# hrnr/map-merge

Hardware: NVIDIA B200
Metric: pairwise_registrations_per_sec (higher is better)
Workload: dtype f32

## Files before the change

map-merge_b200/csrc/icp.cu:

```cuda
#include <algorithm>
#include <cmath>
#include <cstring>
#include <type_traits>

#include "mm3d_internal.cuh"

namespace mm3d {

namespace {

constexpr int IB = 128;
constexpr int NSUM = 17;

struct IcpState {
  float final_t[16];
  float step[16];
  double prev_mse;
  int iterations;
  int active;
  int converged;
  int pad;
};

struct IcpJob {
  GridView tgt;
  ReachView reach;
  const float4* src;
  int ns;
  float4* work;
  long long* sums;
  IcpState* st;
  int* ticket;
  int* next_tile;
  int n_tiles;
  float t0[16];
  long long* sums_log;
  int* nn_slot;
};

struct IcpLoop {
  int n_active;
  int pad[3];
};

struct ReachJob {
  GridView g;
  ReachView r;
  unsigned char* a;
  unsigned char* b;
};

__global__ void __launch_bounds__(256) reach_mark_kernel(const ReachJob* __restrict__ jobs)
{
  const ReachJob& j = jobs[blockIdx.y];
  for (int i = blockIdx.x * blockDim.x + threadIdx.x; i < j.g.n; i += gridDim.x * blockDim.x) {
    const float4 p = j.g.pts[i];
    const int x = floor_to_int(p.x * j.g.inv_leaf) - j.g.min_b[0] - j.r.org[0];
    const int y = floor_to_int(p.y * j.g.inv_leaf) - j.g.min_b[1] - j.r.org[1];
    const int z = floor_to_int(p.z * j.g.inv_leaf) - j.g.min_b[2] - j.r.org[2];
    if (x >= 0 && y >= 0 && z >= 0 && x < j.r.dim[0] && y < j.r.dim[1] && z < j.r.dim[2])
      j.a[((size_t)z * j.r.dim[1] + y) * j.r.dim[0] + x] = 0;
  }
}

__global__ void __launch_bounds__(256) reach_pass_kernel(const ReachJob* __restrict__ jobs, int axis, int margin, int from_a)
{
  const ReachJob& j = jobs[blockIdx.y];
  const size_t ncell = (size_t)j.r.dim[0] * j.r.dim[1] * j.r.dim[2];
  const unsigned char* in = from_a ? j.a : j.b;
  unsigned char* out = from_a ? j.b : j.a;
  for (size_t c = (size_t)blockIdx.x * blockDim.x + threadIdx.x; c < ncell; c += (size_t)gridDim.x * blockDim.x) {
    const int x = (int)(c % j.r.dim[0]);
    const int y = (int)((c / j.r.dim[0]) % j.r.dim[1]);
    const int z = (int)(c / ((size_t)j.r.dim[0] * j.r.dim[1]));
    const int pos = axis == 0 ? x : (axis == 1 ? y : z);
    const int len = j.r.dim[axis];
    const long long stride = axis == 0 ? 1 : (axis == 1 ? (long long)j.r.dim[0] : (long long)j.r.dim[0] * j.r.dim[1]);
    const int lo = max(-margin, -pos), hi = min(margin, len - 1 - pos);
    int best = 255;
    for (int d = lo; d <= hi; ++d) {
      const int f = max(abs(d) - 1, 0);
      const int v = (int)in[(long long)c + (long long)d * stride] + f * f;
      best = min(best, v);
    }
    out[c] = (unsigned char)min(best, j.r.none);
  }
}

__device__ __forceinline__ bool reach_lookup(const GridView& g, const ReachView& r, float qx, float qy, float qz, int* lb2)
{
  const int x = floor_to_int(qx * g.inv_leaf) - g.min_b[0] - r.org[0];
  const int y = floor_to_int(qy * g.inv_leaf) - g.min_b[1] - r.org[1];
  const int z = floor_to_int(qz * g.inv_leaf) - g.min_b[2] - r.org[2];
  if (x < 0 || y < 0 || z < 0 || x >= r.dim[0] || y >= r.dim[1] || z >= r.dim[2]) return false;
  *lb2 = (int)__ldg(&r.lb2[((size_t)z * r.dim[1] + y) * r.dim[0] + x]);
  return true;
}

__device__ __forceinline__ bool reach_descend(const ReachView& r, int& x, int& y, int& z, int cur)
{
  for (int step = 0; step < 48 && cur > 0; ++step) {
    int best = cur, bx = x, by = y, bz = z;
#pragma unroll
    for (int t = 0; t < 6; ++t) {
      const int nx = x + (t == 0) - (t == 1), ny = y + (t == 2) - (t == 3), nz = z + (t == 4) - (t == 5);
      if (nx < 0 || ny < 0 || nz < 0 || nx >= r.dim[0] || ny >= r.dim[1] || nz >= r.dim[2]) continue;
      const int v = (int)__ldg(&r.lb2[((size_t)nz * r.dim[1] + ny) * r.dim[0] + nx]);
      if (v < best) {
        best = v;
        bx = nx;
        by = ny;
        bz = nz;
      }
    }
    if (best >= cur) return false;
    cur = best;
    x = bx;
    y = by;
    z = bz;
  }
  return cur == 0;
}

__device__ __forceinline__ float block27_any(const GridView& g, int vx, int vy, int vz, float qx, float qy, float qz)
{
  float best = 3.0e38f;
  const int xlo = max(vx - 1, 0), xhi = min(vx + 1, g.div_v[0] - 1);
  if (xlo > xhi) return best;
  for (int t = 0; t < 9; ++t) {
    const int cz = vz + t / 3 - 1, cy = vy + t % 3 - 1;
    if (cz < 0 || cz >= g.div_v[2] || cy < 0 || cy >= g.div_v[1]) continue;
    const int base = (cz * g.dim[1] + cy) * g.dim[0];
    const int s = __ldg(&g.cell_start[base + xlo]), e = __ldg(&g.cell_start[base + xhi + 1]);
    for (int k = s; k < e; ++k) {
      const float4 p = g.pts[k];
      best = fminf(best, em::dist2_3(qx, qy, qz, p.x, p.y, p.z));
    }
  }
  return best;
}

__device__ __forceinline__ bool nearest_block27(const GridView& g, float qx, float qy, float qz, double bound, int guess_slot, int* out_idx,
                                                float* out_d2, float4* out_pt, int* out_slot, bool* certain)
{
  const float fx = qx * g.inv_leaf, fy = qy * g.inv_leaf, fz = qz * g.inv_leaf;
  const float flx = floorf(fx), fly = floorf(fy), flz = floorf(fz);
  const int vx = (int)flx - g.min_b[0], vy = (int)fly - g.min_b[1], vz = (int)flz - g.min_b[2];
  const float ay = fy - fly, az = fz - flz;
  bool found = false;
  float best = 0.0f;
  int best_idx = 0x7fffffff, best_slot = -1;
  float4 best_pt = make_float4(0.f, 0.f, 0.f, 0.f);
  float bestv = 3.0e38f;
  const float inv2 = g.inv_leaf * g.inv_leaf;
  if (guess_slot >= 0 && guess_slot < g.n) {
    const float4 p = g.pts[guess_slot];
    const float d2 = em::dist2_3(qx, qy, qz, p.x, p.y, p.z);
    if ((double)d2 <= bound) {
      found = true;
      best = d2;
      best_idx = g.orig ? g.orig[guess_slot] : guess_slot;
      best_slot = guess_slot;
      best_pt = p;
      bestv = d2 * inv2 * 1.0001f + 1e-4f;
    }
  }
  int rs[9], re[9];
  const int xlo = max(vx - 1, 0), xhi = min(vx + 1, g.div_v[0] - 1);
  const bool x_ok = xlo <= xhi;
#pragma unroll
  for (int t = 0; t < 9; ++t) {
    const int cz = vz + t / 3 - 1, cy = vy + t % 3 - 1;
    rs[t] = 0;
    re[t] = 0;
    if (x_ok && cz >= 0 && cz < g.div_v[2] && cy >= 0 && cy < g.div_v[1]) {
      const int base = (cz * g.dim[1] + cy) * g.dim[0];
      rs[t] = __ldg(&g.cell_start[base + xlo]);
      re[t] = __ldg(&g.cell_start[base + xhi + 1]);
    }
  }
#pragma unroll
  for (int t = 0; t < 9; ++t) {
    const int dz = t / 3 - 1, dy = t % 3 - 1;
    const float zd = dz < 0 ? az : (dz > 0 ? 1.0f - az : 0.0f);
    const float yd = dy < 0 ? ay : (dy > 0 ? 1.0f - ay : 0.0f);
    if (zd * zd + yd * yd > bestv) continue;
    for (int k = rs[t]; k < re[t]; ++k) {
      const float4 p = g.pts[k];
      const float d2 = em::dist2_3(qx, qy, qz, p.x, p.y, p.z);
      if ((double)d2 > bound) continue;
      const int oi = g.orig ? g.orig[k] : k;
      if (!found || d2 < best || (d2 == best && oi < best_idx)) {
        found = true;
        best = d2;
        best_idx = oi;
        best_slot = k;
        best_pt = p;
        bestv = d2 * inv2 * 1.0001f + 1e-4f;
      }
    }
  }
  *certain = found && best * inv2 < 0.999f;
  *out_idx = best_idx;
  *out_d2 = best;
  *out_pt = best_pt;
  *out_slot = found ? best_slot : -1;
  return found;
}

struct TileNn {
  float4 q[IB];
  int todo[IB];
  int todo_large[IB];
  float res_d2[IB];
  int res_slot[IB];
  int n_todo, n_todo_large;
};

__device__ __forceinline__ bool tile_nearest(TileNn& sh, const GridView& g, const ReachView& r, bool live, float qx, float qy, float qz,
                                             double bound, int guess_slot, float* out_d2, float4* out_pt, int* out_slot)
{
  const int tid = threadIdx.x, lane = tid & 31, warp = tid >> 5;
  if (tid == 0) {
    sh.n_todo = 0;
    sh.n_todo_large = 0;
  }
  __syncthreads();
  bool hit = false, pending = false;
  float d2 = 0.f;
  int slot = -1;
  float4 pt = make_float4(0.f, 0.f, 0.f, 0.f);
  if (live) {
    float r2 = (float)bound;
    bool rejected = false, block_has_points = true;
    if (r.lb2) {
      int lb2 = 0;
      const float bound_v = (float)bound * g.inv_leaf * g.inv_leaf;
      const bool inside = reach_lookup(g, r, qx, qy, qz, &lb2);
      const float lb = inside ? (float)lb2 : (float)r.none;
      if (lb > bound_v * 1.001f + 0.01f) rejected = true;
      if (inside && lb2 < r.none) {
        const float ub = sqrtf((float)lb2) + 3.4642f;
        r2 = fminf(r2, (ub * ub * 1.001f + 0.01f) * g.leaf * g.leaf);
      }
      block_has_points = inside && lb2 == 0;
      if (!rejected && inside && lb2 > 0 && lb2 < r.none && guess_slot < 0 && g.shift[0] == 0 && g.shift[1] == 0 && g.shift[2] == 0) {
        int cx = floor_to_int(qx * g.inv_leaf) - g.min_b[0] - r.org[0];
        int cy = floor_to_int(qy * g.inv_leaf) - g.min_b[1] - r.org[1];
        int cz = floor_to_int(qz * g.inv_leaf) - g.min_b[2] - r.org[2];
        if (reach_descend(r, cx, cy, cz, lb2)) {
          const float dd = block27_any(g, cx + r.org[0], cy + r.org[1], cz + r.org[2], qx, qy, qz);
          if (dd < 3.0e38f) r2 = fminf(r2, dd);
        }
      }
    }
    if (!rejected) {
      bool certain = false;
      if ((block_has_points || guess_slot >= 0) && g.shift[0] == 0 && g.shift[1] == 0 && g.shift[2] == 0) {
        int idx;
        hit = nearest_block27(g, qx, qy, qz, bound, guess_slot, &idx, &d2, &pt, &slot, &certain);
        if (hit) r2 = fminf(r2, d2);
      }
      if (!certain) {
        pending = true;
        hit = false;
        const float r2w = r2 * 1.00001f + 1e-12f;
        sh.q[tid] = make_float4(qx, qy, qz, r2w);
        if (r2w * g.inv_leaf * g.inv_leaf <= 12.25f) sh.todo[atomicAdd(&sh.n_todo, 1)] = tid;
        else sh.todo_large[atomicAdd(&sh.n_todo_large, 1)] = tid;
      }
    }
  }
  __syncthreads();
  const int n_small = sh.n_todo, n_large = sh.n_todo_large;
  auto serve = [&](auto G_, int who, unsigned gmask, int glane) {
    constexpr int G = decltype(G_)::value;
    const float4 q = sh.q[who];
    const int rv = (int)ceilf(sqrtf(q.w) * g.inv_leaf) + 1;
    float bd = 3.0e38f;
    int bi = 0x7fffffff, bs = -1;
    group_radius_unordered<G>(g, gmask, glane, q.x, q.y, q.z, q.w, rv, [&](bool valid, int k, const float4&, float dd) {
      if (valid && (double)dd <= bound) {
        const int oi = g.orig ? g.orig[k] : k;
        if (dd < bd || (dd == bd && oi < bi)) {
          bd = dd;
          bi = oi;
          bs = k;
        }
      }
    });
#pragma unroll
    for (int o = G / 2; o > 0; o >>= 1) {
      const float od = __shfl_xor_sync(gmask, bd, o, G);
      const int oi = __shfl_xor_sync(gmask, bi, o, G);
      const int os = __shfl_xor_sync(gmask, bs, o, G);
      if (od < bd || (od == bd && oi < bi)) {
        bd = od;
        bi = oi;
        bs = os;
      }
    }
    if (glane == 0) {
      sh.res_d2[who] = bd;
      sh.res_slot[who] = bs;
    }
  };
  {
    const int grp = tid >> 3, glane = tid & 7;
    const unsigned gmask = 0xffu << (lane & 24);
    for (int t = grp; t < n_small; t += IB / 8) serve(std::integral_constant<int, 8>(), sh.todo[t], gmask, glane);
  }
  __syncwarp();
  for (int t = warp; t < n_large; t += IB / 32) serve(std::integral_constant<int, 32>(), sh.todo_large[t], 0xffffffffu, lane);
  __syncthreads();
  if (pending) {
    slot = sh.res_slot[tid];
    hit = slot >= 0;
    if (hit) {
      d2 = sh.res_d2[tid];
      pt = g.pts[slot];
    }
  }
  *out_d2 = d2;
  *out_pt = pt;
  *out_slot = hit ? slot : -1;
  return hit;
}

__global__ void __launch_bounds__(256) icp_init_kernel(const IcpJob* __restrict__ jobs)
{
  const IcpJob& j = jobs[blockIdx.y];
  for (int i = blockIdx.x * blockDim.x + threadIdx.x; i < j.ns; i += gridDim.x * blockDim.x) {
    const float4 p = j.src[i];
    float4 o;
    em::transform_point(j.t0, p.x, p.y, p.z, &o.x, &o.y, &o.z);
    o.w = p.w;
    j.work[i] = o;
    j.nn_slot[i] = -1;
  }
}

__device__ __forceinline__ void block_accumulate(long long* vals, int nvals, long long* gsums)
{
  __shared__ long long sh[IB / 32][NSUM];
  const int lane = threadIdx.x & 31, w = threadIdx.x >> 5;
  __syncthreads();
  for (int k = 0; k < nvals; ++k) {
    const long long v = warp_sum_ll(vals[k]);
    if (lane == 0) sh[w][k] = v;
  }
  __syncthreads();
  if (threadIdx.x < nvals) {
    long long s = 0;
    for (int ww = 0; ww < IB / 32; ++ww) s += sh[ww][threadIdx.x];
    if (s != 0) atomicAdd((unsigned long long*)&gsums[threadIdx.x], (unsigned long long)s);
  }
}

__device__ void mat4_mul(const float* a, const float* b, float* r)
{
  for (int i = 0; i < 4; ++i)
    for (int c = 0; c < 4; ++c) {
      float acc = a[i * 4 + 0] * b[0 * 4 + c];
      acc += a[i * 4 + 1] * b[1 * 4 + c];
      acc += a[i * 4 + 2] * b[2 * 4 + c];
      acc += a[i * 4 + 3] * b[3 * 4 + c];
      r[i * 4 + c] = acc;
    }
}

__device__ void icp_solve(const IcpJob& j, int max_iterations, double rotation_threshold, double translation_threshold, int max_log,
                          int* n_active)
{
  IcpState& st = *j.st;
  long long s[NSUM];
  for (int k = 0; k < NSUM; ++k) {
    s[k] = (long long)atomicExch((unsigned long long*)&j.sums[k], 0ull);
  }
  if (j.sums_log && st.iterations < max_log)
    for (int k = 0; k < NSUM; ++k) j.sums_log[(size_t)st.iterations * NSUM + k] = s[k];
  const long long cnt = s[0];
  if (cnt < 3) {
    st.active = 0;
    st.converged = 0;
    __threadfence();
    atomicSub(n_active, 1);
    return;
  }
  const double n = (double)cnt;
  double pm[3], qm[3];
  for (int a = 0; a < 3; ++a) {
    pm[a] = ((double)s[1 + a] / MM3D_FIX1_SCALE) / n;
    qm[a] = ((double)s[4 + a] / MM3D_FIX1_SCALE) / n;
  }
  float sigma[9], pmf[3], qmf[3];
  for (int a = 0; a < 3; ++a) {
    pmf[a] = (float)pm[a];
    qmf[a] = (float)qm[a];
    for (int b = 0; b < 3; ++b) sigma[a * 3 + b] = (float)(((double)s[7 + a * 3 + b] / MM3D_FIX2_SCALE) / n - qm[a] * pm[b]);
  }
  float T[16];
  em::umeyama_from_sigma<float>(sigma, pmf, qmf, T);
  float nf[16];
  mat4_mul(T, st.final_t, nf);
  for (int k = 0; k < 16; ++k) {
    st.final_t[k] = nf[k];
    st.step[k] = T[k];
  }
  st.iterations += 1;
  bool conv = false;
  if (st.iterations >= max_iterations) {
    conv = true;
  } else {
    const double cos_angle = 0.5 * (double)(T[0] + T[5] + T[10] - 1);
    const double translation_sqr = (double)(T[3] * T[3] + T[7] * T[7] + T[11] * T[11]);
    if (cos_angle >= rotation_threshold && translation_sqr <= translation_threshold) {
      conv = true;
    } else {
      const double mse = ((double)s[16] / MM3D_FIXD_SCALE) / n;
      if (fabs(mse - st.prev_mse) < 1e-12) conv = true;
      else st.prev_mse = mse;
    }
  }
  if (conv) {
    st.active = 0;
    st.converged = 1;
    __threadfence();
    atomicSub(n_active, 1);
  } else {
    __threadfence();
    atomicExch(j.next_tile, 0);
  }
}

__device__ __forceinline__ void icp_tile(const IcpJob& j, int tile, double max_dist_sqr, int rv, int max_iterations,
                                         double rotation_threshold, double translation_threshold, int max_log, int* n_active)
{
  __shared__ float s_step[16];
  __shared__ int s_apply;
  __shared__ TileNn nn;
  __syncthreads();
  if (threadIdx.x < 16) s_step[threadIdx.x] = __ldcg(&j.st->step[threadIdx.x]);
  if (threadIdx.x == 16) s_apply = __ldcg(&j.st->iterations) > 0 ? 1 : 0;
  __syncthreads();
  const int apply_step = s_apply;
  long long v[NSUM];
#pragma unroll
  for (int k = 0; k < NSUM; ++k) v[k] = 0;
  const int i = tile * IB + threadIdx.x;
  const bool live = i < j.ns;
  float4 p = make_float4(0.f, 0.f, 0.f, 0.f);
  int guess = -1;
  if (live) {
    p = __ldcg(&j.work[i]);
    if (apply_step) {
      float4 o;
      em::transform_point(s_step, p.x, p.y, p.z, &o.x, &o.y, &o.z);
      o.w = p.w;
      p = o;
      j.work[i] = p;
    }
    guess = __ldcg(&j.nn_slot[i]);
  }
  float d2;
  float4 q;
  int slot;
  const bool hit = tile_nearest(nn, j.tgt, j.reach, live, p.x, p.y, p.z, max_dist_sqr, guess, &d2, &q, &slot);
  if (live) {
    j.nn_slot[i] = slot;
    if (hit) {
      const double pp[3] = {(double)p.x, (double)p.y, (double)p.z};
      const double qq[3] = {(double)q.x, (double)q.y, (double)q.z};
      v[0] = 1;
#pragma unroll
      for (int a = 0; a < 3; ++a) {
        v[1 + a] = em::to_fix(pp[a], MM3D_FIX1_SCALE);
        v[4 + a] = em::to_fix(qq[a], MM3D_FIX1_SCALE);
#pragma unroll
        for (int b = 0; b < 3; ++b) v[7 + a * 3 + b] = em::to_fix(qq[a] * pp[b], MM3D_FIX2_SCALE);
      }
      v[16] = em::to_fix((double)d2, MM3D_FIXD_SCALE);
    }
  }
  block_accumulate(v, NSUM, j.sums);
  __syncthreads();
  if (threadIdx.x == 0) {
    __threadfence();
    const int ntiles = (j.ns + IB - 1) / IB;
    const int ticket = atomicAdd(j.ticket, 1);
    if (ticket == ntiles - 1) {
      *j.ticket = 0;
      __threadfence();
      icp_solve(j, max_iterations, rotation_threshold, translation_threshold, max_log, n_active);
    }
  }
}

__global__ void __launch_bounds__(IB) icp_persistent_kernel(const IcpJob* __restrict__ jobs, int n_jobs, IcpLoop* loop, double max_dist_sqr,
                                                            int rv, int max_iterations, double rotation_threshold,
                                                            double translation_threshold, int max_log)
{
  __shared__ int s_pair, s_tile;
  int cur = 0;
  for (;;) {
    if (threadIdx.x == 0) {
      int pair = -1, tile = -1, scanned = 0;
      while (__ldcg(&loop->n_active) > 0) {
        const IcpJob& j = jobs[cur];
        if (__ldcg(j.next_tile) < j.n_tiles) {
          const int t = atomicAdd(j.next_tile, 1);
          if (t < j.n_tiles) {
            __threadfence();
            pair = cur;
            tile = t;
            break;
          }
        }
        cur = cur + 1 == n_jobs ? 0 : cur + 1;
        if (++scanned >= n_jobs) {
          scanned = 0;
          __nanosleep(500);
        }
      }
      s_pair = pair;
      s_tile = tile;
    }
    __syncthreads();
    const int pair = s_pair, tile = s_tile;
    if (pair < 0) break;
    icp_tile(jobs[pair], tile, max_dist_sqr, rv, max_iterations, rotation_threshold, translation_threshold, max_log, &loop->n_active);
    __syncthreads();
  }
}

struct ScoreJob {
  GridView tgt;
  ReachView reach;
  const float4* src;
  int ns;
  float t[16];
  long long* sums;
  const int* nn_guess;
};

__global__ void __launch_bounds__(IB) score_kernel(const ScoreJob* __restrict__ jobs, double max_range, int rv)
{
  const ScoreJob& j = jobs[blockIdx.y];
  if (blockIdx.x * IB >= j.ns) return;
  __shared__ TileNn nn;
  long long v[2] = {0, 0};
  const int i = blockIdx.x * IB + threadIdx.x;
  const bool live = i < j.ns;
  float x = 0.f, y = 0.f, z = 0.f;
  if (live) {
    const float4 p = j.src[i];
    em::transform_point(j.t, p.x, p.y, p.z, &x, &y, &z);
  }
  float d2;
  float4 q;
  int slot;
  if (tile_nearest(nn, j.tgt, j.reach, live, x, y, z, max_range, (live && j.nn_guess) ? j.nn_guess[i] : -1, &d2, &q, &slot)) {
    v[0] = em::to_fix((double)d2, MM3D_FIXD_SCALE);
    v[1] = 1;
  }
  block_accumulate(v, 2, j.sums);
}

ReachView no_reach()
{
  ReachView r;
  memset(&r, 0, sizeof(r));
  return r;
}

}

void build_reach_batch(Ctx& c, const std::vector<DIndex>& idx, int margin, std::vector<DReach>& out)
{
  const int M = (int)idx.size();
  out.clear();
  out.resize(M);
  margin = std::max(2, std::min(margin, 15));
  std::vector<ReachJob> jobs;
  std::vector<DBuf<unsigned char>> ping(M);
  size_t max_cells = 0;
  int max_n = 0;
  for (int m = 0; m < M; ++m) {
    out[m].v = no_reach();
    const GridView& g = idx[m].v;
    if (g.n <= 0 || g.div_v[0] <= 0) continue;
    ReachView r = no_reach();
    size_t cells = 1;
    for (int k = 0; k < 3; ++k) {
      r.org[k] = -margin;
      r.dim[k] = g.div_v[k] + 2 * margin;
      cells *= (size_t)r.dim[k];
    }
    if (cells > ((size_t)1 << 30)) continue;
    r.none = std::min(255, margin * margin);
    out[m].lb2.alloc(c, cells);
    ping[m].alloc(c, cells);
    MM_CUDA(cudaMemsetAsync(ping[m].p, 255, cells, c.stream));
    r.lb2 = out[m].lb2.p;
    out[m].v = r;
    jobs.push_back(ReachJob{g, r, ping[m].p, out[m].lb2.p});
    max_cells = std::max(max_cells, cells);
    max_n = std::max(max_n, g.n);
  }
  if (jobs.empty()) return;
  DBuf<ReachJob> dj = to_device(c, jobs);
  const unsigned nj = (unsigned)jobs.size();
  MM_LAUNCH(c, reach_mark_kernel, dim3(std::max(1, std::min((max_n + 255) / 256, 148 * 4)), nj), 256, 0, dj.p);
  const unsigned blocks = (unsigned)std::min<size_t>((max_cells + 255) / 256, 148 * 16);
  double bytes = 0;
  for (const ReachJob& j : jobs) bytes += 2.0 * j.r.dim[0] * j.r.dim[1] * j.r.dim[2];
  MM_BYTES(c, bytes);
  MM_LAUNCH(c, reach_pass_kernel, dim3(blocks, nj), 256, 0, dj.p, 0, margin, 1);
  MM_BYTES(c, bytes);
  MM_LAUNCH(c, reach_pass_kernel, dim3(blocks, nj), 256, 0, dj.p, 1, margin, 0);
  MM_BYTES(c, bytes);
  MM_LAUNCH(c, reach_pass_kernel, dim3(blocks, nj), 256, 0, dj.p, 2, margin, 1);
}

void icp_batch(Ctx& c, const std::vector<CloudView>& clouds, const std::vector<DIndex>& idx, const std::vector<DReach>& reach,
               const std::vector<PairJob>& jobs, const std::vector<const float*>& T0, double max_dist, int max_it, double eps,
               std::vector<IcpOut>& out, std::vector<std::vector<long long>>* sums_dbg, IcpNeighbours* nn_keep)
{
  const int P = (int)jobs.size();
  out.assign(P, IcpOut());
  if (nn_keep) nn_keep->offset.assign(P, -1);
  if (sums_dbg) { sums_dbg->clear(); sums_dbg->resize(P); }
  if (P == 0) return;
  const int max_log = sums_dbg ? 64 : 0;
  std::vector<int> act;
  for (int p = 0; p < P; ++p) {
    bool zero = true;
    for (int k = 0; k < 16; ++k)
      if (T0[p][k] != 0.0f) zero = false;
    if (zero) {
      for (int k = 0; k < 16; ++k) out[p].T[k] = 0.0f;
      out[p].iterations = 0;
      out[p].converged = 0;
    } else {
      act.push_back(p);
    }
  }
  const int A = (int)act.size();
  if (A == 0) return;
  std::stable_sort(act.begin(), act.end(), [&](int x, int y) { return jobs[x].b < jobs[y].b; });
  size_t tot = 0;
  int mx = 0;
  for (int a = 0; a < A; ++a) {
    tot += (size_t)clouds[jobs[act[a]].a].n;
    mx = std::max(mx, clouds[jobs[act[a]].a].n);
  }
  DBuf<float4> work(c, tot + 1);
  DBuf<int> nn_local;
  DBuf<int>& nn = nn_keep ? nn_keep->slots : nn_local;
  nn.alloc(c, tot + 1);
  DBuf<long long> sums(c, (size_t)A * NSUM);
  sums.zero(c);
  DBuf<int> tickets(c, A);
  tickets.zero(c);
  DBuf<long long> slog;
  if (max_log) {
    slog.alloc(c, (size_t)A * max_log * NSUM);
    slog.zero(c);
  }
  std::vector<IcpState> hst(A);
  for (int a = 0; a < A; ++a) {
    memset(&hst[a], 0, sizeof(IcpState));
    for (int k = 0; k < 16; ++k) hst[a].final_t[k] = hst[a].step[k] = (k % 5 == 0) ? 1.f : 0.f;
    hst[a].prev_mse = 1.7976931348623157e308;
    hst[a].active = clouds[jobs[act[a]].a].n > 0 ? 1 : 0;
  }
  DBuf<IcpState> dst = to_device(c, hst);
  std::vector<IcpJob> ij(A);
  size_t off = 0;
  for (int a = 0; a < A; ++a) {
    const PairJob& pj = jobs[act[a]];
    ij[a].tgt = idx[pj.b].v;
    ij[a].reach = pj.b < (int)reach.size() ? reach[pj.b].v : no_reach();
    ij[a].src = clouds[pj.a].pts;
    ij[a].ns = clouds[pj.a].n;
    ij[a].work = work.p + off;
    ij[a].nn_slot = nn.p + off;
    if (nn_keep) nn_keep->offset[act[a]] = (long long)off;
    ij[a].sums = sums.p + (size_t)a * NSUM;
    ij[a].st = dst.p + a;
    ij[a].ticket = tickets.p + a;
    for (int k = 0; k < 16; ++k) ij[a].t0[k] = T0[act[a]][k];
    ij[a].sums_log = max_log ? slog.p + (size_t)a * max_log * NSUM : nullptr;
    off += (size_t)ij[a].ns;
  }
  std::vector<int> hnext(A, 0);
  IcpLoop hl;
  memset(&hl, 0, sizeof(hl));
  int tiles = 0;
  double bytes = 0;
  for (int a = 0; a < A; ++a) {
    ij[a].n_tiles = (ij[a].ns + IB - 1) / IB;
    if (hst[a].active) {
      hl.n_active += 1;
      tiles += ij[a].n_tiles;
      bytes += 16.0 * (2.0 * ij[a].ns + ij[a].tgt.n);
    } else {
      hnext[a] = ij[a].n_tiles;
    }
  }
  DBuf<int> dnext = to_device(c, hnext);
  for (int a = 0; a < A; ++a) ij[a].next_tile = dnext.p + a;
  DBuf<IcpJob> dij = to_device(c, ij);
  DBuf<IcpLoop> dloop(c, 1);
  dloop.upload(c, &hl, 1);
  const int iblocks = std::max(1, std::min((mx + 255) / 256, 148 * 8));
  MM_LAUNCH(c, icp_init_kernel, dim3(iblocks, A), 256, 0, dij.p);
  const double max_dist_sqr = max_dist * max_dist;
  const float leaf = idx[jobs[act[0]].b].v.leaf;
  const int rv = (int)std::ceil(max_dist / (double)leaf) + 1;
  if (hl.n_active > 0) {
    int dev = 0, sms = 0, per_sm = 0;
    MM_CUDA(cudaGetDevice(&dev));
    MM_CUDA(cudaDeviceGetAttribute(&sms, cudaDevAttrMultiProcessorCount, dev));
    MM_CUDA(cudaOccupancyMaxActiveBlocksPerMultiprocessor(&per_sm, icp_persistent_kernel, IB, 0));
    const int grid = std::max(1, std::min(sms * std::max(per_sm, 1), tiles));
    MM_BYTES(c, bytes);
    MM_LAUNCH(c, icp_persistent_kernel, grid, IB, 0, dij.p, A, dloop.p, max_dist_sqr, rv, max_it, 1.0 - eps, eps, max_log);
  }
  dst.download(c, hst.data(), A);
  std::vector<long long> hlog;
  if (max_log) {
    hlog.resize((size_t)A * max_log * NSUM);
    slog.download(c, hlog.data(), hlog.size());
  }
  c.sync();
  for (int a = 0; a < A; ++a) {
    IcpOut& o = out[act[a]];
    const float* f = hst[a].final_t;
    const float* g = T0[act[a]];
    for (int i = 0; i < 4; ++i)
      for (int cc = 0; cc < 4; ++cc) {
        float acc = f[i * 4 + 0] * g[0 * 4 + cc];
        acc += f[i * 4 + 1] * g[1 * 4 + cc];
        acc += f[i * 4 + 2] * g[2 * 4 + cc];
        acc += f[i * 4 + 3] * g[3 * 4 + cc];
        o.T[i * 4 + cc] = acc;
      }
    o.iterations = hst[a].iterations;
    o.converged = hst[a].converged;
    if (sums_dbg) {
      const int nl = std::min(hst[a].iterations + (hst[a].converged ? 0 : 1), max_log);
      (*sums_dbg)[act[a]].assign(hlog.begin() + (size_t)a * max_log * NSUM, hlog.begin() + ((size_t)a * max_log + nl) * NSUM);
    }
  }
}

void score_batch(Ctx& c, const std::vector<CloudView>& clouds, const std::vector<DIndex>& idx, const std::vector<DReach>& reach,
                 const std::vector<PairJob>& jobs, const std::vector<const float*>& T, double max_range, std::vector<double>& scores,
                 const IcpNeighbours* nn_guess)
{
  const int P = (int)jobs.size();
  scores.assign(P, 1.7976931348623157e308);
  if (P == 0) return;
  DBuf<long long> sums(c, (size_t)P * 2);
  sums.zero(c);
  std::vector<ScoreJob> sj(P);
  int mx = 0;
  std::vector<int> ord(P);
  for (int p = 0; p < P; ++p) ord[p] = p;
  std::stable_sort(ord.begin(), ord.end(), [&](int x, int y) { return jobs[x].b < jobs[y].b; });
  for (int q = 0; q < P; ++q) {
    const int p = ord[q];
    sj[q].tgt = idx[jobs[p].b].v;
    sj[q].reach = jobs[p].b < (int)reach.size() ? reach[jobs[p].b].v : no_reach();
    sj[q].src = clouds[jobs[p].a].pts;
    sj[q].ns = clouds[jobs[p].a].n;
    for (int k = 0; k < 16; ++k) sj[q].t[k] = T[p][k];
    sj[q].sums = sums.p + (size_t)p * 2;
    sj[q].nn_guess = (nn_guess && p < (int)nn_guess->offset.size() && nn_guess->offset[p] >= 0) ? nn_guess->slots.p + nn_guess->offset[p] : nullptr;
    mx = std::max(mx, sj[q].ns);
  }
  if (mx == 0) return;
  DBuf<ScoreJob> dsj = to_device(c, sj);
  const float leaf = idx[jobs[0].b].v.leaf;
  const int rv = (int)std::ceil(std::sqrt(std::max(max_range, 0.0)) / (double)leaf) + 1;
  { double b = 0; for (int p = 0; p < P; ++p) b += 16.0 * ((double)sj[p].ns + sj[p].tgt.n); MM_BYTES(c, b); }
  MM_LAUNCH(c, score_kernel, dim3((mx + IB - 1) / IB, P), IB, 0, dsj.p, max_range, rv);
  std::vector<long long> h((size_t)P * 2);
  sums.download(c, h.data(), h.size());
  c.sync();
  for (int p = 0; p < P; ++p)
    if (h[2 * p + 1] > 0) scores[p] = ((double)h[2 * p] / MM3D_FIXD_SCALE) / (double)h[2 * p + 1];
}

}
```

Measured before the change: 1063.

## Tile reach distance passes through shared memory and widen ICP certainty radius

Rewrites the separable reach-distance pass kernel. Each block now stages a line segment plus margin halo in shared memory and applies a compile-time-unrolled tap loop, replacing per-cell strided global reads with coalesced tiled loads. Separately, the nearest_block27 certainty test now uses the query's distance to the nearest voxel face, so more queries count as resolved and skip the fallback search. The block count is rescaled to match, and a profiling script that histograms query distance classes is added.

```diff
diff --git a/map-merge_b200/csrc/icp.cu b/map-merge_b200/csrc/icp.cu
--- a/map-merge_b200/csrc/icp.cu
+++ b/map-merge_b200/csrc/icp.cu
@@ -63,28 +63,60 @@
   }
 }
 
-__global__ void __launch_bounds__(256) reach_pass_kernel(const ReachJob* __restrict__ jobs, int axis, int margin, int from_a)
-{
-  const ReachJob& j = jobs[blockIdx.y];
-  const size_t ncell = (size_t)j.r.dim[0] * j.r.dim[1] * j.r.dim[2];
+constexpr int REACH_MAX_MARGIN = 15;
+
+template <int RW, int M>
+__device__ __forceinline__ int reach_taps(const unsigned char* p, int margin)
+{
+  if constexpr (M > 2) {
+    if (margin < M) return reach_taps<RW, M - 1>(p, margin);
+  }
+  int best = 255;
+#pragma unroll
+  for (int d = -M; d <= M; ++d) {
+    const int f = d < -1 ? -d - 1 : (d > 1 ? d - 1 : 0);
+    best = min(best, (int)p[(M + d) * RW] + f * f);
+  }
+  return best;
+}
+
+template <int RW>
+__device__ __forceinline__ void reach_pass_tiles(const ReachJob& j, int axis, int margin, int from_a, unsigned char* s)
+{
+  constexpr int RL = RW == 1 ? 256 : 64, NY = 256 / RW;
   const unsigned char* in = from_a ? j.a : j.b;
   unsigned char* out = from_a ? j.b : j.a;
-  for (size_t c = (size_t)blockIdx.x * blockDim.x + threadIdx.x; c < ncell; c += (size_t)gridDim.x * blockDim.x) {
-    const int x = (int)(c % j.r.dim[0]);
-    const int y = (int)((c / j.r.dim[0]) % j.r.dim[1]);
-    const int z = (int)(c / ((size_t)j.r.dim[0] * j.r.dim[1]));
-    const int pos = axis == 0 ? x : (axis == 1 ? y : z);
-    const int len = j.r.dim[axis];
-    const long long stride = axis == 0 ? 1 : (axis == 1 ? (long long)j.r.dim[0] : (long long)j.r.dim[0] * j.r.dim[1]);
-    const int lo = max(-margin, -pos), hi = min(margin, len - 1 - pos);
-    int best = 255;
-    for (int d = lo; d <= hi; ++d) {
-      const int f = max(abs(d) - 1, 0);
-      const int v = (int)in[(long long)c + (long long)d * stride] + f * f;
-      best = min(best, v);
-    }
-    out[c] = (unsigned char)min(best, j.r.none);
-  }
+  const long long d0 = j.r.dim[0], d1 = j.r.dim[1], d2 = j.r.dim[2];
+  const int len = j.r.dim[axis];
+  const long long inner = axis == 0 ? 1 : (axis == 1 ? d0 : d0 * d1);
+  const long long outer = axis == 2 ? 1 : (axis == 1 ? d2 : d1 * d2);
+  const long long n_it = (inner + RW - 1) / RW, n_lt = (len + RL - 1) / RL;
+  const long long n_tiles = outer * n_lt * n_it;
+  const int tx = threadIdx.x % RW, ty = threadIdx.x / RW;
+  for (long long t = blockIdx.x; t < n_tiles; t += gridDim.x) {
+    const long long it = t % n_it, lt = (t / n_it) % n_lt, o = t / (n_it * n_lt);
+    const long long i = it * RW + tx;
+    const int l0 = (int)(lt * RL);
+    const long long base = o * len * inner + i;
+    __syncthreads();
+    for (int r = ty; r < RL + 2 * margin; r += NY) {
+      const int l = l0 - margin + r;
+      s[r * RW + tx] = (i < inner && l >= 0 && l < len) ? in[base + (long long)l * inner] : (unsigned char)255;
+    }
+    __syncthreads();
+    if (i >= inner) continue;
+    for (int r = ty; r < RL && l0 + r < len; r += NY) {
+      const int best = reach_taps<RW, REACH_MAX_MARGIN>(s + r * RW + tx, margin);
+      out[base + (long long)(l0 + r) * inner] = (unsigned char)min(best, j.r.none);
+    }
+  }
+}
+
+__global__ void __launch_bounds__(256) reach_pass_kernel(const ReachJob* __restrict__ jobs, int axis, int margin, int from_a)
+{
+  __shared__ unsigned char s[(64 + 2 * REACH_MAX_MARGIN) * 32];
+  if (axis == 0) reach_pass_tiles<1>(jobs[blockIdx.y], axis, margin, from_a, s);
+  else reach_pass_tiles<32>(jobs[blockIdx.y], axis, margin, from_a, s);
 }
 
 __device__ __forceinline__ bool reach_lookup(const GridView& g, const ReachView& r, float qx, float qy, float qz, int* lb2)
@@ -146,7 +178,7 @@
   const float fx = qx * g.inv_leaf, fy = qy * g.inv_leaf, fz = qz * g.inv_leaf;
   const float flx = floorf(fx), fly = floorf(fy), flz = floorf(fz);
   const int vx = (int)flx - g.min_b[0], vy = (int)fly - g.min_b[1], vz = (int)flz - g.min_b[2];
-  const float ay = fy - fly, az = fz - flz;
+  const float ax = fx - flx, ay = fy - fly, az = fz - flz;
   bool found = false;
   float best = 0.0f;
   int best_idx = 0x7fffffff, best_slot = -1;
@@ -200,7 +232,9 @@
       }
     }
   }
-  *certain = found && best * inv2 < 0.999f;
+  const float edge = fminf(fminf(fminf(ax, 1.0f - ax), fminf(ay, 1.0f - ay)), fminf(az, 1.0f - az));
+  const float clear = 1.0f + edge;
+  *certain = found && best * inv2 < clear * clear * 0.999f;
   *out_idx = best_idx;
   *out_d2 = best;
   *out_pt = best_pt;
@@ -233,6 +267,7 @@
   if (live) {
     float r2 = (float)bound;
     bool rejected = false, block_has_points = true;
+    const bool unit = g.shift[0] == 0 && g.shift[1] == 0 && g.shift[2] == 0;
     if (r.lb2) {
       int lb2 = 0;
       const float bound_v = (float)bound * g.inv_leaf * g.inv_leaf;
@@ -244,7 +279,7 @@
         r2 = fminf(r2, (ub * ub * 1.001f + 0.01f) * g.leaf * g.leaf);
       }
       block_has_points = inside && lb2 == 0;
-      if (!rejected && inside && lb2 > 0 && lb2 < r.none && guess_slot < 0 && g.shift[0] == 0 && g.shift[1] == 0 && g.shift[2] == 0) {
+      if (!rejected && inside && lb2 > 0 && lb2 < r.none && guess_slot < 0 && unit) {
         int cx = floor_to_int(qx * g.inv_leaf) - g.min_b[0] - r.org[0];
         int cy = floor_to_int(qy * g.inv_leaf) - g.min_b[1] - r.org[1];
         int cz = floor_to_int(qz * g.inv_leaf) - g.min_b[2] - r.org[2];
@@ -256,7 +291,7 @@
     }
     if (!rejected) {
       bool certain = false;
-      if ((block_has_points || guess_slot >= 0) && g.shift[0] == 0 && g.shift[1] == 0 && g.shift[2] == 0) {
+      if ((block_has_points || guess_slot >= 0) && unit) {
         int idx;
         hit = nearest_block27(g, qx, qy, qz, bound, guess_slot, &idx, &d2, &pt, &slot, &certain);
         if (hit) r2 = fminf(r2, d2);
@@ -580,7 +615,7 @@
   const int M = (int)idx.size();
   out.clear();
   out.resize(M);
-  margin = std::max(2, std::min(margin, 15));
+  margin = std::max(2, std::min(margin, REACH_MAX_MARGIN));
   std::vector<ReachJob> jobs;
   std::vector<DBuf<unsigned char>> ping(M);
   size_t max_cells = 0;
@@ -611,7 +646,7 @@
   DBuf<ReachJob> dj = to_device(c, jobs);
   const unsigned nj = (unsigned)jobs.size();
   MM_LAUNCH(c, reach_mark_kernel, dim3(std::max(1, std::min((max_n + 255) / 256, 148 * 4)), nj), 256, 0, dj.p);
-  const unsigned blocks = (unsigned)std::min<size_t>((max_cells + 255) / 256, 148 * 16);
+  const unsigned blocks = (unsigned)std::min<size_t>((max_cells + 2047) / 2048, 148 * 16);
   double bytes = 0;
   for (const ReachJob& j : jobs) bytes += 2.0 * j.r.dim[0] * j.r.dim[1] * j.r.dim[2];
   MM_BYTES(c, bytes);
diff --git a/profiles/icp_query_classes.py b/profiles/icp_query_classes.py
--- /dev/null
+++ b/profiles/icp_query_classes.py
@@ -0,0 +1,59 @@
+import os
+import sys
+
+import numpy as np
+from scipy.spatial import cKDTree
+
+sys.dont_write_bytecode = True
+sys.path.insert(0, os.path.join(os.path.dirname(os.path.dirname(os.path.abspath(__file__))), "map-merge_b200"))
+import synth
+
+LEAF = 0.1
+M = 6
+
+
+def vox(p):
+    k = np.floor(p[:, :3] / LEAF).astype(np.int64)
+    k -= k.min(0)
+    d = k.max(0) + 1
+    key = (k[:, 2] * d[1] + k[:, 1]) * d[0] + k[:, 0]
+    u, inv, cnt = np.unique(key, return_inverse=True, return_counts=True)
+    c = np.zeros((len(u), 3))
+    np.add.at(c, inv, p[:, :3])
+    return (c / cnt[:, None]).astype(np.float32)
+
+
+def main():
+    maps, truth = synth.make_maps(**dict(synth.CONFIGS["c3"]), only=range(M))
+    V = [vox(maps[m]) for m in range(M)]
+    trees = [cKDTree(v) for v in V]
+    rng = np.random.default_rng(0)
+    for err in (0.0, 0.03, 0.06, 0.1):
+        H = np.zeros(13)
+        nq = 0
+        for a in range(M):
+            for b in range(a + 1, M):
+                T = np.linalg.inv(truth[b]) @ truth[a]
+                ang = np.deg2rad(err * 10)
+                ax = rng.normal(size=3)
+                ax /= np.linalg.norm(ax)
+                K = np.array([[0, -ax[2], ax[1]], [ax[2], 0, -ax[0]], [-ax[1], ax[0], 0]])
+                R = np.eye(3) + np.sin(ang) * K + (1 - np.cos(ang)) * K @ K
+                tv = rng.normal(size=3)
+                tv *= err / np.linalg.norm(tv)
+                P = np.eye(4)
+                P[:3, :3] = R
+                P[:3, 3] = tv
+                T = P @ T
+                q = V[a] @ T[:3, :3].T + T[:3, 3]
+                d, _ = trees[b].query(q, distance_upper_bound=1.0)
+                dv = d / LEAF
+                H += np.histogram(np.where(np.isinf(dv), 12.5, dv), bins=list(range(14)))[0]
+                nq += len(q)
+        h = H / nq
+        print(f"guess error {err:.2f} m / {err * 10:.1f} deg: < 1 voxel {h[0]:.3f}, 1-2 {h[1]:.3f}, 2-10 {h[2:10].sum():.3f}, "
+              f"none within 10 {h[10:].sum():.3f}")
+
+
+if __name__ == "__main__":
+    main()
```

Result: faster. 1081 (median of 6 runs) (+1.7%).
